# bnulwh/gpushare-scheduler-extender

Measured on AMD Instinct MI355X. Metric: pods bound/sec, higher is better.
Workload: dtype n/a

## Files before the change

native/engine/bindings.cc:

```cpp
#include <pybind11/pybind11.h>
#include <pybind11/stl.h>

#include <poll.h>
#include <pthread.h>
#include <sched.h>
#include <sys/eventfd.h>
#include <sys/timerfd.h>
#include <time.h>
#include <unistd.h>

#include <condition_variable>
#include <deque>
#include <memory>
#include <map>
#include <mutex>
#include <thread>

#include "allocstate.h"
#include "dpcore.h"
#include "h2.h"
#include "introspect.h"
#include "ledger.h"
#include "quantity.h"
#include "controller.h"
// ... 475 lines not shown
    d["unfiltered_binds"] = s.unfiltered_binds.load();
    d["live_gets"] = s.live_gets.load();
    d["qps_waits"] = s.qps_waits.load();
    d["moves_failed"] = s.moves_failed.load();
    d["physical_posts"] = s.physical_posts.load();
    d["plugin_auth_denied"] = s.plugin_auth_denied.load();
    d["token_reviews"] = s.token_reviews.load();
    d["backoffs"] = s.backoffs.load();
    d["publication_waits"] = s.publication_waits.load();
    d["physical_refused"] = s.physical_refused.load();
    d["epoch"] = srv_->epoch();
    d["api_throttled"] = srv_->api_throttled();
    d["api_throttle_wait_s"] = srv_->api_throttle_wait_s();
    auto hist = [](const LatencyHist& h) {
      py::dict o;
      py::list bounds, counts;
      for (int i = 0; i < LatencyHist::kBuckets; ++i) bounds.append(LatencyHist::kBounds[i]);
      for (int i = 0; i <= LatencyHist::kBuckets; ++i) counts.append(h.counts[i].load());
      o["bounds"] = bounds;
      o["counts"] = counts;
      o["n"] = h.n.load();
      o["sum"] = static_cast<double>(h.sum_ns.load()) / 1e9;
      return o;
    };
    d["filter_latency"] = hist(s.filter_lat);
    d["bind_latency"] = hist(s.bind_lat);
    d["api_latency"] = hist(s.api_lat);
    return d;
  }

  py::dict ledger_mutex() {
    introspect::MutexStats m = l_.mu().stats();
    py::dict d;
    d["acquisitions"] = m.acquisitions;
    d["contended"] = m.contended;
    d["wait_s"] = m.wait_s;
    d["max_wait_s"] = m.max_wait_s;
    d["hold_s"] = m.hold_s;
    d["max_hold_s"] = m.max_hold_s;
    return d;
  }

  void set_binds_enabled(bool on) {
    binds_enabled_ = on;
    if (srv_) srv_->set_binds_enabled(on);
  }

  py::list drain_annotation_repairs() {
    std::vector<AnnotationRepair> rs;
    {
      std::lock_guard<introspect::ProfiledMutex> g(l_.mu());
      rs = l_.drain_repairs();
    }
    py::list out;
    for (auto& a : rs) {
      py::dict d;
      d["uid"] = a.uid;
      d["namespace"] = a.ns;
      d["name"] = a.name;
      d["node"] = a.node;
      d["dev"] = a.dev;
      d["dev_total"] = a.dev_total;
      d["mem"] = a.mem;
      d["assume_ns"] = a.assume_ns;
      out.append(d);
    }
    return out;
  }

  void set_bind_order(const std::string& m) {
    if (m == "auto") {
      l_.set_order_mode(Ledger::kOrderAuto);
    } else if (m == "strict") {
      l_.set_order_mode(Ledger::kOrderStrict);
    } else if (m == "relaxed") {
      l_.set_order_mode(Ledger::kOrderRelaxed);
    } else {
      throw py::value_error("bind order must be auto, strict or relaxed");
    }
  }
  std::string bind_order() const { return Ledger::order_mode_name(l_.order_mode()); }

  void set_update_mode(bool on) {
    update_mode_ = on;
    if (srv_) srv_->set_update_mode(on);
  }

  py::list drain_bind_failures() {
    py::list out;
    if (!srv_) return out;
    for (auto& f : srv_->drain_failures()) {
      py::dict d;
      d["namespace"] = f.ns;
      d["name"] = f.name;
      d["uid"] = f.uid;
      d["node"] = f.node;
      d["message"] = f.message;
      out.append(d);
    }
    return out;
  }

  size_t pending_count() {
    std::lock_guard<introspect::ProfiledMutex> g(l_.mu());
    return l_.pending_count();
  }

  ~Engine() {
    stop_server();
    stop_controller();
  }

  PodView parse_pod(const py::bytes& b) {
    PodView v;
    std::string err;
    if (!parse_pod_bytes(b, l_.profile(), &v, &err)) throw py::value_error(err);
    return v;
  }

 private:
  Ledger l_;
  bool update_mode_ = false;
  std::unique_ptr<NativeServer> srv_;
  std::unique_ptr<Controller> ctl_;
  bool binds_enabled_ = true;
};

}

namespace {

class PyPodTracker {
 public:
  PyPodTracker(const py::dict& api, const std::string& ns, const std::string& label_selector)
      : t_(api_from(api), ns, label_selector) {}
  void start(double timeout) {
    std::string err;
    bool ok;
    {
      py::gil_scoped_release rel;
      ok = t_.start(timeout, &err);
    }
    if (!ok) throw std::runtime_error(err);
  }
  void stop() {
    py::gil_scoped_release rel;
    t_.stop();
  }
  std::string wait(const std::vector<std::string>& keys, int cond, double timeout) {
    py::gil_scoped_release rel;
    return t_.wait(keys, cond, timeout);
  }
  size_t size() const { return t_.size(); }

 private:
  PodTracker t_;
};

class PyReflectorProbe {
 public:
  PyReflectorProbe(const py::dict& api, const std::string& path, const std::string& field_selector, int page) {
    ReflectorConfig rc;
    rc.path = path;
    rc.field_selector = field_selector;
    rc.list_page_size = page;
    ReflectorHandler h;
    h.on_list = [this](const ListView& lv) {
      std::map<std::string, std::string> fresh;
      for (size_t k = 0; k < lv.size(); ++k) {
        std::string key, rv;
        if (key_rv(lv.doc(k), lv.obj(k), &key, &rv)) fresh[key] = rv;
      }
      std::lock_guard<std::mutex> g(mu_);
      view_.swap(fresh);
      lists_++;
    };
    h.on_event = [this](Ev ev, const json::Doc& d, uint32_t obj) {
      std::string key, rv;
      if (!key_rv(d, obj, &key, &rv)) return;
      std::lock_guard<std::mutex> g(mu_);
      if (ev == Ev::Deleted) {
        view_.erase(key);
      } else {
        view_[key] = rv;
      }
      events_++;
    };
    r_ = std::make_unique<Reflector>(api_from(api), rc, h);
  }
  ~PyReflectorProbe() { stop(); }
  void start() { r_->start(); }
  void stop() {
    if (r_) {
      py::gil_scoped_release rel;
      r_->stop();
    }
  }
  bool wait_synced(double t) {
    py::gil_scoped_release rel;
    return r_->wait_synced(t);
  }
  void request_relist() { r_->request_relist(); }
  py::dict view() {
    py::dict d;
    std::lock_guard<std::mutex> g(mu_);
    for (auto& kv : view_) d[py::str(kv.first)] = kv.second;
    return d;
  }
  py::dict stats() {
    py::dict d;
    d["relists"] = r_->relists();
    d["rewatches"] = r_->rewatches();
    d["errors"] = r_->errors();
    d["resource_version"] = r_->resource_version();
    std::lock_guard<std::mutex> g(mu_);
    d["lists"] = lists_;
    d["events"] = events_;
    return d;
  }

 private:
  static bool key_rv(const json::Doc& d, uint32_t obj, std::string* key, std::string* rv) {
    int64_t n = d.path(obj, {"metadata", "name"});
    if (n < 0) return false;
    int64_t ns = d.path(obj, {"metadata", "namespace"});
    int64_t r = d.path(obj, {"metadata", "resourceVersion"});
    *key = (ns >= 0 ? d.str(static_cast<uint32_t>(ns)) + "/" : std::string()) + d.str(static_cast<uint32_t>(n));
    *rv = r >= 0 ? d.str(static_cast<uint32_t>(r)) : std::string();
    return true;
  }
  std::unique_ptr<Reflector> r_;
  std::mutex mu_;
  std::map<std::string, std::string> view_;
  uint64_t lists_ = 0, events_ = 0;
};

class PyBatchClient {
 public:
  explicit PyBatchClient(const py::dict& api) : c_(api_from(api)) {}
  py::list run(const std::vector<std::tuple<std::string, std::string, py::bytes>>& reqs, int concurrency) {
    std::vector<std::tuple<std::string, std::string, std::string>> rq;
    rq.reserve(reqs.size());
    for (const auto& r : reqs) rq.emplace_back(std::get<0>(r), std::get<1>(r), std::string(std::get<2>(r)));
    std::vector<std::pair<int, std::string>> out;
    {
      py::gil_scoped_release rel;
      out = c_.run(rq, concurrency);
    }
    py::list l;
    for (auto& o : out) l.append(py::make_tuple(o.first, py::bytes(o.second)));
    return l;
  }

 private:
  BatchClient c_;
};

py::dict open_loop_run(const py::dict& api, const std::string& run, const std::string& pod_tmpl, double rate,
                       double duration_s, double warm_s, double hold_s, double drain_s, int creators, int deleters,
                       const std::string& ns, int grace) {
  OpenLoopConfig c;
  c.grace = grace;
  c.run = run;
  c.pod_tmpl = pod_tmpl;
  c.rate = rate;
  c.duration_s = duration_s;
  c.warm_s = warm_s;
  c.hold_s = hold_s;
  c.drain_s = drain_s;
  c.creators = creators;
  c.deleters = deleters;
  c.ns = ns;
  OpenLoop ol(api_from(api));
  std::vector<OpenLoopPod> pods;
  std::string err;
  int ce = 0, de = 0;
  bool ok;
  {
    py::gil_scoped_release rel;
    ok = ol.run(c, &pods, &err, &ce, &de);
  }
  if (!ok) throw std::runtime_error(err);
  py::list l;
  for (const auto& p : pods) l.append(py::make_tuple(p.arrival, p.created, p.bound, p.running, p.deleted, p.gone, p.failed));
  py::dict d;
  d["pods"] = l;
  d["create_errors"] = ce;
  d["delete_errors"] = de;
  return d;
}

class PyPodRuntime {
 public:
  PyPodRuntime(int dev, uint64_t arena_bytes, uint64_t arena_addr, uint64_t stream, uint64_t stride,
               const std::string& kernels_lib) {
    PodRuntimeConfig c;
    c.dev = dev;
    c.arena_bytes = arena_bytes;
    c.arena_addr = arena_addr;
    c.stream = reinterpret_cast<void*>(stream);
    c.stride = stride;
    c.kernels_lib = kernels_lib;
    r_ = std::make_unique<PodRuntime>(c);
    std::string err;
    if (!r_->init(&err)) throw std::runtime_error(err);
  }
// ... 727 lines not shown
  std::mutex fmu_;
  std::vector<Feed> feed_;
  std::vector<Waiting> waiting_;
  uint64_t waited_ = 0, feed_events_ = 0;
  double wait_s_ = 0, wait_max_s_ = 0;
  int tfd_ = -1;
  std::vector<std::thread> workers_;
  std::mutex wmu_;
  std::condition_variable wcv_;
  std::deque<std::unique_ptr<DpPending>> todo_, done_;
  std::deque<std::unique_ptr<DpPending>> todo_bg_;
  bool stopping_ = false;
  bool serving_on_ = false;
  int efd_ = -1;
  std::unique_ptr<DpCore> core_;
  std::unique_ptr<h2::Server> srv_;
  std::vector<std::tuple<uint64_t, std::string, std::string>> pending_;
  std::vector<DpEvent> events_;
  std::string device_list_, last_why_;
  bool have_list_ = false, fast_ = true;
  std::thread serving_;
  std::atomic<bool> stop_serving_{false};
  int pyfd_ = -1;
  double h_pref_s_ = 0, h_alloc_s_ = 0, h_pref_max_ = 0, h_alloc_max_ = 0;
  bool ready_ = true;
  bool preferred_ = false;
  double py_event_s_ = 0.002;
  double py_signal_at_ = 0, py_due_ = 0;
  bool py_deferred_ = false;
  double lock_wait_s_ = 0, lock_wait_max_s_ = 0;
  uint64_t lock_waits_ = 0;
  uint64_t h_pref_n_ = 0, h_alloc_n_ = 0;
  double spin_us_ = 1000;
  uint64_t calls_seen_ = 0;
  uint64_t spins_ = 0;
  uint64_t loop_iters_ = 0, spin_iters_ = 0;
  uint64_t passes_ = 0;
};

PYBIND11_MODULE(_engine, m) {
  m.def(
      "native_symbol", [](uint64_t pc) { return introspect::symbol_at(static_cast<uintptr_t>(pc)); },
      "Function name at a program counter of this process ('' when unknown).");
  m.def(
      "native_stacks",
      [](std::vector<int> tids, double timeout) {
        std::vector<introspect::Sample> got;
        {
          py::gil_scoped_release rel;
          got = introspect::capture(tids, timeout);
        }
        py::list out;
        for (auto& smp : got) out.append(py::make_tuple(smp.tid, smp.comm, smp.ok, smp.frames));
        return out;
      },
      py::arg("tids") = std::vector<int>(), py::arg("timeout") = 0.05,
      "Stack samples (tid, comm, ok, frames innermost-first) of this process's threads (all when tids is empty).");

  m.doc() = "gpushare MI355X native ledger engine";

  py::class_<PodView>(m, "PodView")
      .def(py::init<>())
      .def_readwrite("uid", &PodView::uid)
      .def_readwrite("name", &PodView::name)
      .def_readwrite("namespace", &PodView::ns)
      .def_readwrite("node", &PodView::node)
      .def_readwrite("phase", &PodView::phase)
      .def_readwrite("resource_version", &PodView::rv)
      .def_readwrite("deleting", &PodView::deleting)
      .def_readwrite("request", &PodView::request)
      .def_readwrite("dev_idx", &PodView::dev_idx)
      .def_readwrite("annot_mem", &PodView::annot_mem)
      .def_readwrite("has_annot_mem", &PodView::has_annot_mem)
      .def_readwrite("annot_dev_total", &PodView::annot_dev_total)
      .def_readwrite("assigned", &PodView::assigned)
      .def_readwrite("assume_time", &PodView::assume_time)
      .def_readwrite("cu_mask", &PodView::cu_mask)
      .def_readwrite("hold_idx", &PodView::hold_idx)
      .def_property_readonly("terminal", &PodView::terminal)
      .def_property_readonly("complete", &PodView::complete)
      .def_property_readonly("assigned_non_terminated", &PodView::assigned_non_terminated)
      .def("__repr__", [](const PodView& v) {
        return "<PodView " + v.ns + "/" + v.name + " uid=" + v.uid + " node=" + v.node +
               " req=" + std::to_string(v.request) + " idx=" + std::to_string(v.dev_idx) + ">";
      });

  py::class_<Engine>(m, "Engine")
      .def(py::init<const py::dict&>(), py::arg("profile") = py::dict())
      .def("profile", &Engine::profile)
      .def("upsert_node", &Engine::upsert_node, py::arg("name"), py::arg("total"), py::arg("count"),
           py::arg("dev_totals") = std::vector<int64_t>(), py::arg("address") = std::string())
      .def("upsert_node_json", &Engine::upsert_node_json)
      .def("remove_node", &Engine::remove_node)
      .def("has_node", &Engine::has_node)
      .def("node_info", &Engine::node_info)
      .def("upsert_pod", &Engine::upsert_pod)
      .def("remove_pod", &Engine::remove_pod)
      .def("known", &Engine::known)
      .def("pod_state", &Engine::pod_state)
      .def("upsert_pod_json", &Engine::upsert_pod_json)
      .def("check", &Engine::check)
      .def("filter", &Engine::filter)
      .def("prioritize", &Engine::prioritize)
      .def("assume", &Engine::assume)
      .def("finish_bind", &Engine::finish_bind, py::arg("uid"), py::arg("ok"), py::arg("ttl") = 30.0)
      .def("gc", &Engine::gc, py::arg("list_start") = 0.0)
      .def("assume_ordered", &Engine::assume_ordered, py::arg("uid"), py::arg("ns"), py::arg("name"),
           py::arg("node"), py::arg("req"), py::arg("cu_count") = std::string())
      .def("bind_blocked", &Engine::bind_blocked)
      .def("bind_wait", &Engine::bind_wait)
      .def("bind_leave", &Engine::bind_leave)
      .def("controller_gc", &Engine::controller_gc)
      .def("inspect", &Engine::inspect, py::arg("node") = std::string())
      .def("node_devices", &Engine::node_devices)
      .def("node_names", &Engine::node_names)
      .def("stats", &Engine::stats)
      .def("parse_pod", &Engine::parse_pod)
      .def("serve", &Engine::serve, py::arg("host"), py::arg("port"), py::arg("threads") = 2,
           py::arg("pool_threads") = 16, py::arg("fallback_port") = 0, py::arg("ttl") = 60.0,
           py::arg("api") = py::dict(), py::arg("update_mode") = false, py::arg("qps") = 0.0, py::arg("burst") = 10,
           py::arg("plugin_auth") = "none", py::arg("plugin_users") = std::vector<std::string>())
      .def("node_unaccounted", [](Engine& e, const std::string& node) { return e.node_unaccounted(node); })
      .def("begin_move", &Engine::begin_move, py::arg("uid"), py::arg("node"), py::arg("from_dev"), py::arg("to") = -1,
           py::arg("partner") = std::string(), py::arg("physical_on_to") = false, py::arg("req_hold") = -1,
           py::arg("req_hold_partner") = std::string())
      .def("end_move", &Engine::end_move)
      .def("set_unaccounted", &Engine::set_unaccounted, py::arg("node"), py::arg("extra"), py::arg("ttl") = 60.0)
      .def("begin_epoch", &Engine::begin_epoch)
      .def("publication_wait", &Engine::publication_wait)
      .def("stop_server", &Engine::stop_server)
      .def("start_controller", &Engine::start_controller, py::arg("api"), py::arg("resync") = 30.0,
           py::arg("sync_timeout") = 60.0, py::arg("watch_timeout") = 300)
      .def("stop_controller", &Engine::stop_controller)
      .def("controller_synced", &Engine::controller_synced)
      .def("controller_get_pod", &Engine::controller_get_pod)
      .def("controller_overcommitted", &Engine::controller_overcommitted)
      .def("controller_stats", &Engine::controller_stats)
      .def("server_stats", &Engine::server_stats)
      .def("ledger_mutex", &Engine::ledger_mutex)
      .def("drain_bind_failures", &Engine::drain_bind_failures)
      .def("set_binds_enabled", &Engine::set_binds_enabled)
      .def("set_update_mode", &Engine::set_update_mode)
      .def("set_bind_order", &Engine::set_bind_order)
      .def_property_readonly("bind_order", &Engine::bind_order)
      .def("drain_annotation_repairs", &Engine::drain_annotation_repairs)
      .def("pending_count", &Engine::pending_count);

  py::class_<PyPodTracker>(m, "PodTracker")
      .def(py::init<const py::dict&, const std::string&, const std::string&>(), py::arg("api"),
           py::arg("namespace") = std::string(), py::arg("label_selector") = std::string())
      .def("start", &PyPodTracker::start, py::arg("timeout") = 30.0)
      .def("stop", &PyPodTracker::stop)
      .def("wait", &PyPodTracker::wait, py::arg("keys"), py::arg("cond"), py::arg("timeout") = 120.0)
      .def("size", &PyPodTracker::size);
  m.attr("TRACK_BOUND") = static_cast<int>(PodTracker::Bound);
  m.attr("TRACK_RUNNING") = static_cast<int>(PodTracker::Running);
  m.attr("TRACK_GONE") = static_cast<int>(PodTracker::Gone);
  m.attr("TRACK_STOPPED") = static_cast<int>(PodTracker::Stopped);
  py::class_<PyReflectorProbe>(m, "ReflectorProbe")
      .def(py::init<const py::dict&, const std::string&, const std::string&, int>(), py::arg("api"),
           py::arg("path") = "/api/v1/pods", py::arg("field_selector") = "", py::arg("page") = 500)
      .def("start", &PyReflectorProbe::start)
      .def("stop", &PyReflectorProbe::stop)
      .def("wait_synced", &PyReflectorProbe::wait_synced, py::arg("timeout") = 10.0)
      .def("request_relist", &PyReflectorProbe::request_relist)
      .def("view", &PyReflectorProbe::view)
      .def("stats", &PyReflectorProbe::stats);

  m.def("open_loop_run", &open_loop_run, py::arg("api"), py::arg("run"), py::arg("pod_tmpl"), py::arg("rate"),
        py::arg("duration_s") = 2.0, py::arg("warm_s") = 0.5, py::arg("hold_s") = 0.0, py::arg("drain_s") = 20.0,
        py::arg("creators") = 16, py::arg("deleters") = 16, py::arg("ns") = "default", py::arg("grace") = -1);
  py::class_<PyBatchClient>(m, "BatchClient")
      .def(py::init<const py::dict&>())
      .def("run", &PyBatchClient::run, py::arg("requests"), py::arg("concurrency") = 8);

  py::class_<PyPodRuntime>(m, "PodRuntime")
      .def(py::init<int, uint64_t, uint64_t, uint64_t, uint64_t, const std::string&>(), py::arg("dev"),
           py::arg("arena_bytes"), py::arg("arena_addr") = 0, py::arg("stream") = 0, py::arg("stride") = 1 << 20,
           py::arg("kernels_lib") = std::string())
      .def("serve", &PyPodRuntime::serve, py::arg("host") = "127.0.0.1", py::arg("port") = 0,
           py::arg("cpus") = std::vector<int>())
      .def("stop", &PyPodRuntime::stop)
      .def("admit", &PyPodRuntime::admit, py::arg("uid"), py::arg("bytes"), py::arg("verify") = true)
      .def("release", &PyPodRuntime::release)
      .def("verify", &PyPodRuntime::verify)
      .def("stats", &PyPodRuntime::stats);


  py::class_<CuPartitioner>(m, "CuPartitioner")
      .def(py::init<int, int>(), py::arg("cu_count") = 256, py::arg("xcc_count") = 8)
      .def("allocate", [](CuPartitioner& c, const std::string& uid, int n) {
             std::vector<int> out;
             std::string err;
             if (!c.allocate(uid, n, &out, &err)) throw py::value_error(err);
             return out;
           }, py::call_guard<AllocLock>())
      .def("release", &CuPartitioner::release, py::call_guard<AllocLock>())
      .def("adopt", &CuPartitioner::adopt, py::call_guard<AllocLock>())
      .def("swap_owners", &CuPartitioner::swap_owners, py::call_guard<AllocLock>())
      .def("holds", &CuPartitioner::holds, py::call_guard<AllocLock>())
      .def("held_by", &CuPartitioner::held_by, py::call_guard<AllocLock>())
      .def("held", [](const CuPartitioner& c) {
        py::dict d;
        for (const auto& kv : c.held()) d[py::str(kv.first)] = kv.second;
        return d;
      }, py::call_guard<AllocLock>())
      .def("free_count", &CuPartitioner::free_count, py::call_guard<AllocLock>())
      .def_property_readonly("cu_count", &CuPartitioner::cu_count)
      .def_property_readonly("xcc_count", &CuPartitioner::xcc_count);
  m.def("cu_words", &cu_words, py::call_guard<AllocLock>());
  m.def("parse_cu_words", [](const std::string& w) {
    try {
      return parse_cu_words(w);
    } catch (const std::invalid_argument& e) {
      throw py::value_error(e.what());
    }
  }, py::call_guard<AllocLock>());
  m.def("cu_ranges", &cu_ranges, py::call_guard<AllocLock>());

  py::class_<AllocPod>(m, "AllocPod")
      .def(py::init<>())
      .def_readwrite("uid", &AllocPod::uid)
      .def_readwrite("key", &AllocPod::key)
      .def_readwrite("namespace", &AllocPod::ns)
      .def_readwrite("name", &AllocPod::name)
      .def_readwrite("rv", &AllocPod::rv)
      .def_readwrite("phase", &AllocPod::phase)
      .def_readwrite("creation", &AllocPod::creation)
      .def_readwrite("node", &AllocPod::node)
      .def_readwrite("dev", &AllocPod::dev)
      .def_readwrite("request", &AllocPod::request)
      .def_readwrite("containers", &AllocPod::containers)
      .def_readwrite("assume_time", &AllocPod::assume_time)
      .def_readwrite("dev_total", &AllocPod::dev_total)
      .def_readwrite("assigned", &AllocPod::assigned)
      .def_readwrite("complete", &AllocPod::complete)
      .def_readwrite("terminating", &AllocPod::terminating)
      .def_readwrite("term_grace_s", &AllocPod::term_grace_s)
      .def_readwrite("cu_count", &AllocPod::cu_count)
      .def_readwrite("cu_mask", &AllocPod::cu_mask)
      .def_readwrite("hold_idx", &AllocPod::hold_idx)
      .def_readwrite("hold_partner", &AllocPod::hold_partner)
      .def_readwrite("raw", &AllocPod::raw)
      .def_property_readonly("pending", &AllocPod::pending);

  auto rec_dict = [](const AllocRecord& r) {
    py::dict d;
    d["aid"] = r.aid;
    d["ids"] = r.ids;
    d["uid"] = r.uid;
    d["dev"] = r.dev;
    d["units"] = r.units;
    d["cu_mask"] = r.cu_mask;
    d["owner"] = r.owner;
    d["t"] = r.t;
    d["iso"] = r.iso;
    d["on_gpu"] = r.on_gpu;
    return d;
  };
  py::class_<AllocState>(m, "AllocState")
      .def(py::init([](const std::string& node, const std::vector<std::tuple<int, int, int>>& devs) {
             std::vector<std::pair<int, std::pair<int, int>>> d;
             for (const auto& t : devs) d.push_back({std::get<0>(t), {std::get<1>(t), std::get<2>(t)}});
             return new AllocState(node, d);
           }),
           py::arg("node"), py::arg("devices"))
      .def("observe", &AllocState::observe, py::call_guard<AllocLock>())
      .def("release", &AllocState::release, py::call_guard<AllocLock>())
      .def("deleted", &AllocState::deleted, py::arg("uid"), py::arg("now") = -1.0, py::call_guard<AllocLock>())
      .def("lingering", &AllocState::lingering, py::call_guard<AllocLock>())
      .def("gone_held", &AllocState::gone_held, py::call_guard<AllocLock>())
      .def("set_linger", &AllocState::set_linger, py::call_guard<AllocLock>())
      .def("set_skip_partners", &AllocState::set_skip_partners, py::call_guard<AllocLock>())
      .def("linger_enabled", &AllocState::linger_enabled, py::call_guard<AllocLock>())
      .def("linger_count", &AllocState::linger_count, py::call_guard<AllocLock>())
      .def("is_tombstoned", &AllocState::is_tombstoned, py::call_guard<AllocLock>())
      .def("resync", [](AllocState& s, const std::vector<std::string>& live, double now) {
        s.resync(std::unordered_set<std::string>(live.begin(), live.end()), now);
      }, py::arg("live"), py::arg("now") = -1.0, py::call_guard<AllocLock>())
      .def("holders", &AllocState::holders, py::call_guard<AllocLock>())
      .def("has_pod", [](const AllocState& s, const std::string& uid) { return s.pod(uid) != nullptr; }, py::call_guard<AllocLock>())
      .def("uid_for_key", [](const AllocState& s, const std::string& key) -> std::string {
        const AllocPod* p = s.pod_by_key(key);
        return p ? p->uid : std::string();
      }, py::call_guard<AllocLock>())
      .def("pod_view", [](const AllocState& s, const std::string& uid) -> py::object {
             const AllocPod* p = s.pod(uid);
             if (!p) return py::none();
             py::dict d;
             d["rv"] = p->rv;
             d["phase"] = p->phase;
             d["dev"] = p->dev;
             d["assigned"] = p->assigned;
             d["cu_mask"] = p->cu_mask;
             d["hold_idx"] = p->hold_idx;
             d["hold_partner"] = p->hold_partner;
             return d;
           }, py::call_guard<AllocLock>())
      .def("pod_views", [](const AllocState& s) {
        std::vector<AllocPod> copy;
        {
          AllocLock lock;
          copy.resize(s.pods().size());
          size_t i = 0;
          for (const auto& kv : s.pods()) {
            const AllocPod& p = kv.second;
            AllocPod& c = copy[i++];
// ... 244 lines not shown
```

native/engine/podruntime.cc:

```cpp
#include "podruntime.h"

#include <dlfcn.h>

#include <algorithm>
#include <cstdio>
#include <set>
#include <vector>

#include "json.h"

namespace gsx {

namespace {

constexpr uint64_t kAlign = 2ull << 20;

uint64_t tag_of(const std::string& uid) {
  uint64_t h = 1469598103934665603ull;
  for (unsigned char c : uid) {
    h ^= c;
    h *= 1099511628211ull;
  }
  return h | 1;
}

struct GsxSlice {
  uint64_t addr, bytes, tag;
};

}

PodRuntime::PodRuntime(PodRuntimeConfig cfg) : cfg_(std::move(cfg)) {}

PodRuntime::~PodRuntime() {
  stop();
  if (lib_) dlclose(lib_);
}

bool PodRuntime::init(std::string* err) {
  if (!cfg_.arena_addr) return true;
  lib_ = dlopen(cfg_.kernels_lib.c_str(), RTLD_NOW | RTLD_LOCAL);
  if (!lib_) {
    *err = std::string("dlopen ") + cfg_.kernels_lib + ": " + dlerror();
    return false;
  }
  set_device_ = reinterpret_cast<int (*)(int)>(dlsym(lib_, "gsx_set_device"));
  admit_n_ = reinterpret_cast<int (*)(void*, const void*, int, int, int, uint64_t, uint64_t*)>(
      dlsym(lib_, "gsx_hbm_admit_n"));
  last_error_ = reinterpret_cast<const char* (*)()>(dlsym(lib_, "gsx_last_error"));
  if (!set_device_ || !admit_n_ || !last_error_) {
    *err = "libgsx_kernels.so lacks gsx_set_device / gsx_hbm_admit_n";
    return false;
  }
  if (!cfg_.stream || cfg_.stride < 16 || cfg_.stride % 16) {
    *err = "pod runtime needs a stream and a 16-B multiple stamp stride";
    return false;
  }
  return true;
}

int PodRuntime::serve(const std::string& host, int port, std::string* err, std::vector<int> cpus) {
  srv_ = std::make_unique<CtlServer>([this](const http::Message& m) { return handle(m); });
  srv_->set_cpus(std::move(cpus));
  return srv_->start(host, port, err);
}

void PodRuntime::stop() {
  if (srv_) srv_->stop();
}

uint64_t PodRuntime::resident_bytes() const {
  std::lock_guard<std::mutex> g(mu_);
  uint64_t b = 0;
  for (auto& kv : slices_) b += kv.second.size;
  return b;
}

size_t PodRuntime::resident() const {
  std::lock_guard<std::mutex> g(mu_);
  return slices_.size();
}

int64_t PodRuntime::run_admit(bool stamp, const std::string& uid, bool verify, std::string* err) {
  if (!cfg_.arena_addr) return 0;
  std::vector<GsxSlice> sl;
  auto add = [&](const Slice& s) {
    for (auto& e : s.ext) sl.push_back(GsxSlice{cfg_.arena_addr + e.first, e.second, s.tag});
  };
  auto mine = slices_.find(uid);
  if (mine != slices_.end()) add(mine->second);
  const int n_stamp = stamp ? static_cast<int>(sl.size()) : 0;
  if (verify) {
    for (auto& kv : slices_) {
      if (kv.first != uid) add(kv.second);
    }
  }
  if (sl.empty()) return 0;
  uint64_t bad = 0;
  int rc = set_device_(cfg_.dev);
  if (rc == 0) rc = admit_n_(cfg_.stream, sl.data(), static_cast<int>(sl.size()), n_stamp, 1, cfg_.stride, &bad);
  if (rc != 0) {
    *err = std::string("gsx_hbm_admit_n: ") + last_error_();
    return -1;
  }
  return static_cast<int64_t>(bad);
}

bool PodRuntime::carve_locked(const std::string& uid, uint64_t bytes, std::string* err) {
  uint64_t size = (bytes + kAlign - 1) / kAlign * kAlign;
  std::vector<std::pair<uint64_t, uint64_t>> used;
  for (auto& kv : slices_) used.insert(used.end(), kv.second.ext.begin(), kv.second.ext.end());
  std::sort(used.begin(), used.end());
  Slice s{{}, size, tag_of(uid)};
  uint64_t pos = 0, need = size;
  auto take = [&](uint64_t end) {
    if (need && end > pos) {
      uint64_t n = std::min(need, end - pos);
      s.ext.emplace_back(pos, n);
      need -= n;
    }
  };
  for (auto& u : used) {
    take(u.first);
    pos = std::max(pos, u.first + u.second);
  }
  take(cfg_.arena_bytes);
  if (need) {
    *err = "arena exhausted: need " + std::to_string(size) + " B, " + std::to_string(size - need) + " free of " +
           std::to_string(cfg_.arena_bytes);
    return false;
  }
  slices_[uid] = std::move(s);
  return true;
}

void PodRuntime::admit_group_locked(const std::vector<Pending*>& group) {
  std::vector<Pending*> fresh, again;
  bool verify_all = false;
  for (Pending* p : group) {
    if (slices_.count(p->uid)) {
      again.push_back(p);
    } else if (!carve_locked(p->uid, p->bytes, &p->err)) {
      failed_++;
      p->result = -1;
      continue;
    } else {
      fresh.push_back(p);
    }
    verify_all = verify_all || p->verify;
  }
  if (fresh.empty() && again.empty()) return;
  std::vector<GsxSlice> sl;
  std::set<std::string> listed;
  for (Pending* p : fresh) {
    for (auto& e : slices_[p->uid].ext) sl.push_back(GsxSlice{cfg_.arena_addr + e.first, e.second, slices_[p->uid].tag});
    listed.insert(p->uid);
  }
  const int n_stamp = static_cast<int>(sl.size());
  for (auto& kv : slices_) {
    if (listed.count(kv.first)) continue;
    bool own = false;
    for (Pending* p : again) own = own || p->uid == kv.first;
    if (!verify_all && !own) continue;
    for (auto& e : kv.second.ext) sl.push_back(GsxSlice{cfg_.arena_addr + e.first, e.second, kv.second.tag});
  }
  uint64_t bad = 0;
  int rc = 0;
  if (cfg_.arena_addr && !sl.empty()) {
    rc = set_device_(cfg_.dev);
    if (rc == 0) rc = admit_n_(cfg_.stream, sl.data(), static_cast<int>(sl.size()), n_stamp, 1, cfg_.stride, &bad);
    batches_++;
  }
  if (rc != 0) {
    std::string e = std::string("gsx_hbm_admit_n: ") + last_error_();
    for (Pending* p : fresh) {
      slices_.erase(p->uid);
      failed_++;
      p->result = -1;
      p->err = e;
    }
    for (Pending* p : again) {
      p->result = -1;
      p->err = e;
    }
    return;
  }
  bad_ += bad;
  auto own_bad = [&](Pending* p) -> int64_t {
    if (p->verify || bad == 0) return static_cast<int64_t>(bad);
    std::vector<GsxSlice> mine;
    auto it = slices_.find(p->uid);
    if (it == slices_.end()) return 0;
    for (auto& e : it->second.ext) mine.push_back(GsxSlice{cfg_.arena_addr + e.first, e.second, it->second.tag});
    uint64_t b = 0;
    if (!mine.empty() && admit_n_(cfg_.stream, mine.data(), static_cast<int>(mine.size()), 0, 1, cfg_.stride, &b) != 0) {
      return static_cast<int64_t>(bad);
    }
    return static_cast<int64_t>(b);
  };
  for (Pending* p : fresh) {
    admitted_++;
    p->result = own_bad(p);
  }
  for (Pending* p : again) p->result = own_bad(p);
}

int64_t PodRuntime::admit(const std::string& uid, uint64_t bytes, bool verify, std::string* err) {
  Pending me{uid, bytes, verify};
  std::unique_lock<std::mutex> q(qmu_);
  queue_.push_back(&me);
  while (!me.done) {
    if (leading_) {
      qcv_.wait(q);
      continue;
    }
    leading_ = true;
    std::vector<Pending*> group;
    group.swap(queue_);
    q.unlock();
    try {
      std::lock_guard<std::mutex> g(mu_);
      admit_group_locked(group);
    } catch (const std::exception& e) {
      for (Pending* p : group) {
        if (p->result >= 0 && p->err.empty()) {
          p->result = -1;
          p->err = std::string("admission: ") + e.what();
        }
      }
    }
    q.lock();
    for (Pending* p : group) p->done = true;
    leading_ = false;
    qcv_.notify_all();
  }
  if (me.result < 0) *err = me.err;
  return me.result;
}

bool PodRuntime::release(const std::string& uid) {
  std::lock_guard<std::mutex> g(mu_);
  return slices_.erase(uid) > 0;
}

int64_t PodRuntime::verify_all(std::string* err) {
  std::lock_guard<std::mutex> g(mu_);
  return run_admit(false, std::string(), true, err);
}

CtlServer::Reply PodRuntime::handle(const http::Message& m) {
  CtlServer::Reply rep;
  std::string_view path = m.path();
  const std::string_view pre = "/v1/pods/";
  if (path.substr(0, pre.size()) == pre && path.size() > pre.size()) {
    std::string uid(path.substr(pre.size()));
    if (m.method == "POST") {
      json::Doc d;
      std::string err;
      int64_t bytes = 0;
      bool verify = true;
      if (d.parse(m.body, &err)) {
        int64_t b = d.find(0, "bytes");
        if (b >= 0) d.as_int(static_cast<uint32_t>(b), &bytes);
        int64_t v = d.find(0, "verify");
        if (v >= 0) verify = d.at(static_cast<uint32_t>(v)).type != json::T::False;
      }
      if (bytes <= 0) {
        rep.status = 400;
        rep.body = "{\"error\":\"bytes must be > 0\"}";
        return rep;
      }
      int64_t bad = admit(uid, static_cast<uint64_t>(bytes), verify, &err);
      if (bad < 0) {
        rep.status = 409;
        rep.body = "{\"error\":";
        json::append_quoted(&rep.body, err);
        rep.body.push_back('}');
        return rep;
      }
      rep.body = "{\"bad\":" + std::to_string(bad) + "}";
      return rep;
    }
    if (m.method == "DELETE") {
      rep.status = release(uid) ? 200 : 404;
      return rep;
    }
  }
  if (m.method == "GET" && path == "/v1/stats") {
    std::lock_guard<std::mutex> g(mu_);
    char b[256];
    std::snprintf(b, sizeof(b),
                  "{\"admitted\":%llu,\"failed\":%llu,\"bad\":%llu,\"resident\":%zu,\"batches\":%llu,\"native\":true}",
                  (unsigned long long)admitted_, (unsigned long long)failed_, (unsigned long long)bad_,
                  slices_.size(), (unsigned long long)batches_);
    rep.body = b;
    return rep;
  }
  rep.status = 404;
  rep.body = "{\"error\":\"not found\"}";
  return rep;
}

}
```

native/engine/podruntime.h:

```cpp
#pragma once

#include <cstdint>
#include <condition_variable>
#include <map>
#include <memory>
#include <mutex>
#include <string>
#include <utility>
#include <vector>

#include "ctlserver.h"

namespace gsx {

struct PodRuntimeConfig {
  int dev = 0;
  uint64_t arena_bytes = 0;
  uint64_t arena_addr = 0;
  void* stream = nullptr;
  uint64_t stride = 1 << 20;
  std::string kernels_lib;
};

class PodRuntime {
 public:
  explicit PodRuntime(PodRuntimeConfig cfg);
  ~PodRuntime();
  bool init(std::string* err);
  int serve(const std::string& host, int port, std::string* err, std::vector<int> cpus = {});
  void stop();
  int64_t admit(const std::string& uid, uint64_t bytes, bool verify, std::string* err);
  bool release(const std::string& uid);
  int64_t verify_all(std::string* err);
  uint64_t admitted() const { return admitted_; }
  uint64_t failed() const { return failed_; }
  uint64_t bad() const { return bad_; }
  uint64_t batches() const { return batches_; }
  uint64_t resident_bytes() const;
  size_t resident() const;

 private:
  struct Slice {
    std::vector<std::pair<uint64_t, uint64_t>> ext;
    uint64_t size, tag;
  };
  CtlServer::Reply handle(const http::Message& m);
  int64_t run_admit(bool stamp, const std::string& uid, bool verify, std::string* err);
  struct Pending {
    std::string uid;
    uint64_t bytes;
    bool verify;
    bool done = false;
    int64_t result = 0;
    std::string err;
  };
  bool carve_locked(const std::string& uid, uint64_t bytes, std::string* err);
  void admit_group_locked(const std::vector<Pending*>& group);

  PodRuntimeConfig cfg_;
  mutable std::mutex mu_;
  std::map<std::string, Slice> slices_;
  uint64_t admitted_ = 0, failed_ = 0, bad_ = 0, batches_ = 0;
  std::mutex qmu_;
  std::condition_variable qcv_;
  std::vector<Pending*> queue_;
  bool leading_ = false;
  std::unique_ptr<CtlServer> srv_;
  void* lib_ = nullptr;
  int (*set_device_)(int) = nullptr;
  int (*admit_n_)(void*, const void*, int, int, int, uint64_t, uint64_t*) = nullptr;
  const char* (*last_error_)() = nullptr;
};

}
```

native/engine/tracker.cc:

```cpp
#include "tracker.h"

#include <algorithm>
#include <atomic>
#include <chrono>
#include <deque>
#include <thread>
#include <unordered_set>

namespace gsx {

namespace {

std::string str_at(const json::Doc& d, int64_t i) { return i >= 0 ? d.str(static_cast<uint32_t>(i)) : std::string(); }

}

PodTracker::PodTracker(const ApiConfig& cfg, const std::string& ns, const std::string& label_selector) {
  ReflectorConfig rc;
  rc.path = ns.empty() ? "/api/v1/pods" : "/api/v1/namespaces/" + ns + "/pods";
  rc.label_selector = label_selector;
  ReflectorHandler h;
  auto key_of = [](const json::Doc& d, uint32_t obj) {
    std::string ns_ = str_at(d, d.path(obj, {"metadata", "namespace"}));
    std::string name = str_at(d, d.path(obj, {"metadata", "name"}));
    return ns_.empty() ? name : ns_ + "/" + name;
  };
  h.on_list = [this, key_of](const ListView& lv) {
    std::lock_guard<std::mutex> g(mu_);
    pods_.clear();
    for (size_t k = 0; k < lv.size(); ++k) {
      const json::Doc& d = lv.doc(k);
      uint32_t i = lv.obj(k);
      St& s = pods_[key_of(d, i)];
      s.node = str_at(d, d.path(i, {"spec", "nodeName"}));
      s.phase = str_at(d, d.path(i, {"status", "phase"}));
    }
    cv_.notify_all();
  };
  h.on_event = [this, key_of](Ev ev, const json::Doc& d, uint32_t obj) {
    std::string key = key_of(d, obj);
    std::lock_guard<std::mutex> g(mu_);
    if (ev == Ev::Deleted) {
      pods_.erase(key);
    } else {
      St& s = pods_[key];
      s.node = str_at(d, d.path(obj, {"spec", "nodeName"}));
      s.phase = str_at(d, d.path(obj, {"status", "phase"}));
    }
    cv_.notify_all();
  };
  r_ = std::make_unique<Reflector>(cfg, rc, h);
}

PodTracker::~PodTracker() { stop(); }

bool PodTracker::start(double timeout_s, std::string* err) {
  r_->start();
  if (!r_->wait_synced(timeout_s)) {
    *err = "tracker did not sync: " + r_->last_error();
    return false;
  }
  return true;
}

void PodTracker::stop() {
  if (r_) r_->stop();
  cv_.notify_all();
}

size_t PodTracker::size() const {
  std::lock_guard<std::mutex> g(mu_);
  return pods_.size();
}

bool PodTracker::ok_locked(const std::string& key, int cond, std::string* err) const {
  auto it = pods_.find(key);
  switch (cond) {
    case Bound:
      return it != pods_.end() && !it->second.node.empty();
    case Running:
      if (it != pods_.end() && it->second.phase == "Failed") *err = "pod " + key + " Failed";
      return it != pods_.end() && it->second.phase == "Running";
    case Stopped:
      return it == pods_.end() || it->second.phase == "Succeeded" || it->second.phase == "Failed";
    default:
      return it == pods_.end();
  }
}

std::string PodTracker::wait(const std::vector<std::string>& keys, int cond, double timeout_s) {
  auto deadline = std::chrono::steady_clock::now() + std::chrono::duration<double>(timeout_s);
  std::unique_lock<std::mutex> lk(mu_);
  size_t i = 0;
  while (true) {
    std::string err;
    while (i < keys.size() && ok_locked(keys[i], cond, &err)) ++i;
    if (!err.empty()) return err;
    if (i == keys.size()) return std::string();
    if (cv_.wait_until(lk, deadline) == std::cv_status::timeout) {
      while (i < keys.size() && ok_locked(keys[i], cond, &err)) ++i;
      if (i == keys.size()) return std::string();
      return "timeout: " + std::to_string(keys.size() - i) + " pods not " +
             (cond == Bound ? "bound" : cond == Running ? "Running" : cond == Stopped ? "stopped" : "gone") + ", e.g. " + keys[i];
    }
  }
}

BatchClient::~BatchClient() {
  {
    std::lock_guard<std::mutex> g(mu_);
    stop_ = true;
  }
  cv_.notify_all();
  for (auto& t : helpers_) t.join();
}

void BatchClient::work_on(const std::vector<Req>& reqs, std::vector<std::pair<int, std::string>>* out) {
  while (true) {
    size_t i = next_.fetch_add(1);
    if (i >= reqs.size()) return;
    int status = 0;
    std::string body, err;
    const auto& r = reqs[i];
    if (api_.request(std::get<0>(r), std::get<1>(r), std::get<2>(r), "application/json", &status, &body, &err)) {
      (*out)[i] = {status, std::move(body)};
    } else {
      (*out)[i] = {-1, err};
    }
  }
}

void BatchClient::helper(int me) {
  uint64_t seen = 0;
  std::unique_lock<std::mutex> lk(mu_);
  while (true) {
    cv_.wait(lk, [&] { return stop_ || (gen_ != seen && me < want_); });
    if (stop_) return;
    seen = gen_;
    const std::vector<Req>* reqs = reqs_;
    auto* out = out_;
    ++busy_;
    lk.unlock();
    work_on(*reqs, out);
    lk.lock();
    if (--busy_ == 0) done_cv_.notify_all();
  }
}

std::vector<std::pair<int, std::string>> BatchClient::run(const std::vector<Req>& reqs, int concurrency) {
  std::lock_guard<std::mutex> one(run_mu_);
  std::vector<std::pair<int, std::string>> out(reqs.size());
  const int n = std::max(1, std::min<int>(concurrency, static_cast<int>(reqs.size())));
  {
    std::lock_guard<std::mutex> g(mu_);
    while (static_cast<int>(helpers_.size()) < n - 1) {
      const int k = static_cast<int>(helpers_.size());
      helpers_.emplace_back([this, k] { helper(k); });
    }
    reqs_ = &reqs;
    out_ = &out;
    next_.store(0);
    want_ = n - 1;
    ++gen_;
  }
  if (n > 1) cv_.notify_all();
  work_on(reqs, &out);
  std::unique_lock<std::mutex> lk(mu_);
  done_cv_.wait(lk, [&] { return busy_ == 0; });
  want_ = 0;
  reqs_ = nullptr;
  out_ = nullptr;
  return out;
}

}

namespace gsx {

namespace {
double mono() { return std::chrono::duration<double>(std::chrono::steady_clock::now().time_since_epoch()).count(); }
}

bool OpenLoop::run(const OpenLoopConfig& c, std::vector<OpenLoopPod>* pods, std::string* err, int* create_errors,
                   int* delete_errors) {
  const size_t n = static_cast<size_t>(std::max(1.0, c.rate * c.duration_s));
  pods->assign(n, OpenLoopPod{});
  std::mutex mu;
  std::condition_variable cv;
  std::deque<std::pair<double, size_t>> dq;
  std::atomic<int> cerr{0}, derr{0};
  std::atomic<size_t> next{0}, gone{0};
  std::atomic<bool> stop{false};
  const std::string prefix = "ol-" + c.run + "-";
  auto index_of = [&](const json::Doc& d, uint32_t obj) -> int64_t {
    std::string name = str_at(d, d.path(obj, {"metadata", "name"}));
    if (name.compare(0, prefix.size(), prefix) != 0) return -1;
    char* e = nullptr;
    long long i = std::strtoll(name.c_str() + prefix.size(), &e, 10);
    return (e && *e == '\0' && i >= 0 && static_cast<size_t>(i) < n) ? i : -1;
  };
  auto observe = [&](Ev ev, const json::Doc& d, uint32_t obj) {
    int64_t i = index_of(d, obj);
    if (i < 0) return;
    const double now = mono();
    std::lock_guard<std::mutex> g(mu);
    OpenLoopPod& p = (*pods)[static_cast<size_t>(i)];
    if (ev == Ev::Deleted) {
      if (p.gone == 0) {
        p.gone = now;
        gone.fetch_add(1);
        cv.notify_all();
      }
      return;
    }
    if (p.bound == 0 && !str_at(d, d.path(obj, {"spec", "nodeName"})).empty()) p.bound = now;
    std::string phase = str_at(d, d.path(obj, {"status", "phase"}));
    if (p.running == 0 && (phase == "Running" || phase == "Failed")) {
      p.running = now;
      p.failed = phase == "Failed";
      dq.emplace_back(now + c.hold_s, static_cast<size_t>(i));
      cv.notify_all();
    }
  };
  ReflectorConfig rc;
  rc.path = "/api/v1/namespaces/" + c.ns + "/pods";
  rc.label_selector = c.label_key + "=" + c.run;
  ReflectorHandler h;
  h.on_list = [&](const ListView& lv) {
    for (size_t k = 0; k < lv.size(); ++k) observe(Ev::Modified, lv.doc(k), lv.obj(k));
  };
  h.on_event = [&](Ev ev, const json::Doc& d, uint32_t obj) { observe(ev, d, obj); };
  Reflector r(cfg_, rc, h);
  r.start();
  if (!r.wait_synced(30)) {
    *err = "open-loop watch did not sync: " + r.last_error();
    r.stop();
    return false;
  }
  const std::string coll = "/api/v1/namespaces/" + c.ns + "/pods";
  const double t0 = mono() + 0.01;
  std::vector<std::thread> th;
  for (int k = 0; k < std::max(1, c.creators); ++k) {
    th.emplace_back([&] {
      ApiClient api(cfg_);
      std::string body, resp, e;
      while (!stop.load()) {
        size_t i = next.fetch_add(1);
        if (i >= n) return;
        const double at = t0 + static_cast<double>(i) / c.rate;
        const double wait = at - mono();
        if (wait > 0) std::this_thread::sleep_for(std::chrono::duration<double>(wait));
        body = c.pod_tmpl;
// ... 62 lines not shown
```

native/engine/tracker.h:

```cpp
#pragma once

#include <atomic>
#include <condition_variable>
#include <memory>
#include <mutex>
#include <string>
#include <thread>
#include <tuple>
#include <unordered_map>
#include <vector>

#include "apiclient.h"
#include "informer.h"

namespace gsx {

class PodTracker {
 public:
  enum Cond : int { Bound = 0, Running = 1, Gone = 2, Stopped = 3 };
  PodTracker(const ApiConfig& cfg, const std::string& ns, const std::string& label_selector);
  ~PodTracker();
  bool start(double timeout_s, std::string* err);
  void stop();
  std::string wait(const std::vector<std::string>& keys, int cond, double timeout_s);
  size_t size() const;

 private:
  struct St {
    std::string node, phase;
  };
  bool ok_locked(const std::string& key, int cond, std::string* err) const;

  std::unique_ptr<Reflector> r_;
  mutable std::mutex mu_;
  std::condition_variable cv_;
  std::unordered_map<std::string, St> pods_;
};

struct OpenLoopConfig {
  std::string ns = "default";
  std::string label_key = "gsx-ol";
  std::string run;
  std::string pod_tmpl;
  double rate = 1000;
  double duration_s = 2.0;
  double warm_s = 0.5;
  double hold_s = 0.0;
  double drain_s = 20.0;
  int creators = 16, deleters = 16;
  int grace = -1;
};

struct OpenLoopPod {
  double arrival = 0, created = 0, bound = 0, running = 0, deleted = 0, gone = 0;
  bool failed = false;
};

class OpenLoop {
 public:
  explicit OpenLoop(const ApiConfig& cfg) : cfg_(cfg) {}
  bool run(const OpenLoopConfig& c, std::vector<OpenLoopPod>* pods, std::string* err, int* create_errors,
           int* delete_errors);

 private:
  ApiConfig cfg_;
};

class BatchClient {
 public:
  using Req = std::tuple<std::string, std::string, std::string>;
  explicit BatchClient(const ApiConfig& cfg) : api_(cfg) {}
  ~BatchClient();
  std::vector<std::pair<int, std::string>> run(const std::vector<Req>& reqs, int concurrency);

 private:
  void work_on(const std::vector<Req>& reqs, std::vector<std::pair<int, std::string>>* out);
  void helper(int me);

  ApiClient api_;
  std::mutex run_mu_, mu_;
  std::condition_variable cv_, done_cv_;
  std::vector<std::thread> helpers_;
  const std::vector<Req>* reqs_ = nullptr;
  std::vector<std::pair<int, std::string>>* out_ = nullptr;
  std::atomic<size_t> next_{0};
  uint64_t gen_ = 0;
  int want_ = 0, busy_ = 0;
  bool stop_ = false;
};

}
```

native/kernels/hbm_stamp.hip:

```cpp
#include <hip/hip_runtime.h>

#include <algorithm>
#include <mutex>

#include "gsx_internal.h"
#include "gsx_kernels.h"

using namespace gsx;

namespace {

struct alignas(16) Stamp {
  uint64_t tag;
  uint64_t off;
};
typedef unsigned long long u64x2 __attribute__((ext_vector_type(2)));

typedef const __attribute__((address_space(1))) u64x2* global_stamp_ptr;

typedef __attribute__((address_space(1))) u64x2* global_stamp_wptr;

__device__ __forceinline__ u64x2 load_stamp(const char* p) { return *(global_stamp_ptr)(p); }
__device__ __forceinline__ void store_stamp(char* p, uint64_t tag, uint64_t off) {
  u64x2 v;
  v.x = tag;
  v.y = off;
  *(global_stamp_wptr)(p) = v;
}

__device__ __forceinline__ void stamp_extent(const gsx_slice sl, uint64_t stride) {
  const uint64_t n = sl.bytes / stride;
  char* base = reinterpret_cast<char*>(sl.addr);
  for (uint64_t i = blockIdx.x * 256ull + threadIdx.x; i < n; i += gridDim.x * 256ull) {
    store_stamp(base + i * stride, sl.tag, i * stride);
  }
}

__device__ __forceinline__ void count_bad_stamps(const gsx_slice sl, uint64_t stride, unsigned long long* bad) {
  const uint64_t n = sl.bytes / stride;
  const char* base = reinterpret_cast<const char*>(sl.addr);
  uint32_t mine = 0;
  for (uint64_t i = blockIdx.x * 256ull + threadIdx.x; i < n; i += gridDim.x * 256ull) {
    const u64x2 st = load_stamp(base + i * stride);
    mine += (st.x != sl.tag || st.y != i * stride) ? 1u : 0u;
  }
  for (int o = 32; o > 0; o >>= 1) mine += __shfl_xor(mine, o, 64);
  if ((threadIdx.x & 63) == 0 && mine) atomicAdd_system(bad, static_cast<unsigned long long>(mine));
}

constexpr int kMaxSlices = 32;
struct SliceTable {
  gsx_slice s[kMaxSlices];
  int n;
};

__global__ __launch_bounds__(256) void stamp_slices_kernel(SliceTable t, uint64_t stride) {
  stamp_extent(t.s[blockIdx.y], stride);
}

__global__ __launch_bounds__(256) void verify_slices_kernel(SliceTable t, uint64_t stride, unsigned long long* bad) {
  count_bad_stamps(t.s[blockIdx.y], stride, bad);
}


std::mutex g_mu;
unsigned long long* g_host_counter[kMaxDevices] = {nullptr};
std::mutex g_dev_mu[kMaxDevices];

int pinned_counter(const char* who, int* dev, unsigned long long** hc) {
  if (int rc = current_device(who, dev)) return rc;
  std::lock_guard<std::mutex> g(g_mu);
  if (!g_host_counter[*dev]) {
    GSX_CHECK(hipHostMalloc(reinterpret_cast<void**>(&g_host_counter[*dev]), 64, hipHostMallocCoherent));
  }
  *hc = g_host_counter[*dev];
  return 0;
}

constexpr int kTableBlocks = 1024, kRangeBlocks = 8192;

int launch(const char* who, hipStream_t st, const gsx_slice* slices, int n_stamp, int n_verify, uint64_t stride,
           int max_blocks, bool sync, uint64_t* bad) {
  auto tables = [&](int count, auto&& kernel) {
    for (int from = 0; from < count; from += kMaxSlices) {
      SliceTable t;
      t.n = std::min(kMaxSlices, count - from);
      uint64_t maxn = 0;
      for (int i = 0; i < t.n; ++i) {
        t.s[i] = slices[from + i];
        maxn = std::max<uint64_t>(maxn, t.s[i].bytes / stride);
      }
      const uint64_t gx = std::clamp<uint64_t>((maxn + 255) / 256, 1, max_blocks);
      kernel(dim3(static_cast<uint32_t>(gx), t.n), t);
      GSX_CHECK(hipGetLastError());
    }
    return 0;
  };
  if (int rc = tables(n_stamp, [&](dim3 grid, const SliceTable& t) {
        hipLaunchKernelGGL(stamp_slices_kernel, grid, dim3(256), 0, st, t, stride);
      }))
    return rc;
  if (!n_verify) {
    if (sync) GSX_CHECK(hipStreamSynchronize(st));
    return 0;
  }
  int dev = 0;
  unsigned long long* hc = nullptr;
  if (int rc = pinned_counter(who, &dev, &hc)) return rc;
  std::lock_guard<std::mutex> dl(g_dev_mu[dev]);
  __atomic_store_n(hc, 0ull, __ATOMIC_SEQ_CST);
  if (int rc = tables(n_verify, [&](dim3 grid, const SliceTable& t) {
        hipLaunchKernelGGL(verify_slices_kernel, grid, dim3(256), 0, st, t, stride, hc);
      }))
    return rc;
  GSX_CHECK(hipStreamSynchronize(st));
  *bad = __atomic_load_n(hc, __ATOMIC_SEQ_CST);
  return 0;
}

}

extern "C" {

int gsx_hbm_stamp(void* stream, void* base, uint64_t bytes, uint64_t stride, uint64_t tag) {
  if (!base || stride < sizeof(Stamp) || stride % 16) return fail_arg("gsx_hbm_stamp: stride must be >=16, %16");
  if (reinterpret_cast<uintptr_t>(base) % 16) return fail_arg("gsx_hbm_stamp: base not 16-B aligned");
  if (bytes < stride) return 0;
  const gsx_slice sl = {reinterpret_cast<uintptr_t>(base), bytes, tag};
  return launch("gsx_hbm_stamp", S(stream), &sl, 1, 0, stride, kRangeBlocks, false, nullptr);
}

int gsx_hbm_verify(void* stream, const void* base, uint64_t bytes, uint64_t stride, uint64_t tag, uint64_t* bad) {
  if (!base || stride < sizeof(Stamp) || stride % 16) return fail_arg("gsx_hbm_verify: stride must be >=16, %16");
  if (reinterpret_cast<uintptr_t>(base) % 16) return fail_arg("gsx_hbm_verify: base not 16-B aligned");
  *bad = 0;
  if (bytes < stride) return 0;
  const gsx_slice sl = {reinterpret_cast<uintptr_t>(base), bytes, tag};
  return launch("gsx_hbm_verify", S(stream), &sl, 0, 1, stride, kRangeBlocks, true, bad);
}

int gsx_hbm_admit_n(void* stream, const gsx_slice* slices, int n, int n_stamp, int verify, uint64_t stride,
                    uint64_t* bad) {
  *bad = 0;
  if (n < 0 || n_stamp < 0 || n_stamp > n || stride < sizeof(Stamp) || stride % 16)
    return fail_arg("gsx_hbm_admit_n: bad n/n_stamp/stride");
  for (int i = 0; i < n; ++i) {
    if (!slices[i].addr || slices[i].addr % 16) return fail_arg("gsx_hbm_admit_n: slice base not 16-B aligned");
  }
  return launch("gsx_hbm_admit_n", S(stream), slices, n_stamp, verify ? n : 0, stride, kTableBlocks, true, bad);
}

}
```

Baseline: 11680.

## Release runtime lock during GPU admit and wake tracker waiters selectively

PodRuntime now drops its state mutex while the HBM admit kernel runs and caches the selected device per endpoint thread, so it no longer calls set_device on every batch. PodTracker records which keys waiters are blocked on and notifies the condition variable only when an event satisfies or errors one of them, replacing a notify_all on every event. The pinned-counter lookup becomes a lock-free atomic fast path. Event and wakeup counters are also exposed through the Python bindings. Releasing mu_ mid-admit lets other threads change slices_ concurrently, which adds a risk of races.

```diff
diff --git a/native/engine/bindings.cc b/native/engine/bindings.cc
--- a/native/engine/bindings.cc
+++ b/native/engine/bindings.cc
@@ -651,6 +651,13 @@
     return t_.wait(keys, cond, timeout);
   }
   size_t size() const { return t_.size(); }
+  py::dict stats() const {
+    PodTracker::Stats s = t_.stats();
+    py::dict d;
+    d["events"] = s.events;
+    d["wakeups"] = s.wakeups;
+    return d;
+  }
 
  private:
   PodTracker t_;
@@ -1684,7 +1691,8 @@
       .def("start", &PyPodTracker::start, py::arg("timeout") = 30.0)
       .def("stop", &PyPodTracker::stop)
       .def("wait", &PyPodTracker::wait, py::arg("keys"), py::arg("cond"), py::arg("timeout") = 120.0)
-      .def("size", &PyPodTracker::size);
+      .def("size", &PyPodTracker::size)
+      .def("stats", &PyPodTracker::stats);
   m.attr("TRACK_BOUND") = static_cast<int>(PodTracker::Bound);
   m.attr("TRACK_RUNNING") = static_cast<int>(PodTracker::Running);
   m.attr("TRACK_GONE") = static_cast<int>(PodTracker::Gone);
diff --git a/native/engine/podruntime.cc b/native/engine/podruntime.cc
--- a/native/engine/podruntime.cc
+++ b/native/engine/podruntime.cc
@@ -27,6 +27,9 @@
 struct GsxSlice {
   uint64_t addr, bytes, tag;
 };
+
+thread_local bool t_endpoint = false;
+thread_local int t_dev = -1;
 
 }
 
@@ -134,7 +137,7 @@
   return true;
 }
 
-void PodRuntime::admit_group_locked(const std::vector<Pending*>& group) {
+void PodRuntime::admit_group(const std::vector<Pending*>& group, std::unique_lock<std::mutex>& lk) {
   std::vector<Pending*> fresh, again;
   bool verify_all = false;
   for (Pending* p : group) {
@@ -166,13 +169,19 @@
   }
   uint64_t bad = 0;
   int rc = 0;
+  std::string e;
   if (cfg_.arena_addr && !sl.empty()) {
-    rc = set_device_(cfg_.dev);
+    lk.unlock();
+    if (!t_endpoint || t_dev != cfg_.dev) {
+      rc = set_device_(cfg_.dev);
+      t_dev = rc == 0 ? cfg_.dev : -1;
+    }
     if (rc == 0) rc = admit_n_(cfg_.stream, sl.data(), static_cast<int>(sl.size()), n_stamp, 1, cfg_.stride, &bad);
+    if (rc != 0) e = std::string("gsx_hbm_admit_n: ") + last_error_();
+    lk.lock();
     batches_++;
   }
   if (rc != 0) {
-    std::string e = std::string("gsx_hbm_admit_n: ") + last_error_();
     for (Pending* p : fresh) {
       slices_.erase(p->uid);
       failed_++;
@@ -219,8 +228,8 @@
     group.swap(queue_);
     q.unlock();
     try {
-      std::lock_guard<std::mutex> g(mu_);
-      admit_group_locked(group);
+      std::unique_lock<std::mutex> g(mu_);
+      admit_group(group, g);
     } catch (const std::exception& e) {
       for (Pending* p : group) {
         if (p->result >= 0 && p->err.empty()) {
@@ -250,6 +259,7 @@
 
 CtlServer::Reply PodRuntime::handle(const http::Message& m) {
   CtlServer::Reply rep;
+  t_endpoint = true;
   std::string_view path = m.path();
   const std::string_view pre = "/v1/pods/";
   if (path.substr(0, pre.size()) == pre && path.size() > pre.size()) {
diff --git a/native/engine/podruntime.h b/native/engine/podruntime.h
--- a/native/engine/podruntime.h
+++ b/native/engine/podruntime.h
@@ -55,7 +55,7 @@
     std::string err;
   };
   bool carve_locked(const std::string& uid, uint64_t bytes, std::string* err);
-  void admit_group_locked(const std::vector<Pending*>& group);
+  void admit_group(const std::vector<Pending*>& group, std::unique_lock<std::mutex>& lk);
 
   PodRuntimeConfig cfg_;
   mutable std::mutex mu_;
diff --git a/native/engine/tracker.cc b/native/engine/tracker.cc
--- a/native/engine/tracker.cc
+++ b/native/engine/tracker.cc
@@ -47,7 +47,14 @@
       s.node = str_at(d, d.path(obj, {"spec", "nodeName"}));
       s.phase = str_at(d, d.path(obj, {"status", "phase"}));
     }
-    cv_.notify_all();
+    ++events_;
+    for (const Awaited& a : awaited_) {
+      std::string err;
+      if (*a.key == key && (ok_locked(key, a.cond, &err) || !err.empty())) {
+        cv_.notify_all();
+        break;
+      }
+    }
   };
   r_ = std::make_unique<Reflector>(cfg, rc, h);
 }
@@ -71,6 +78,11 @@
 size_t PodTracker::size() const {
   std::lock_guard<std::mutex> g(mu_);
   return pods_.size();
+}
+
+PodTracker::Stats PodTracker::stats() const {
+  std::lock_guard<std::mutex> g(mu_);
+  return Stats{events_, wakeups_};
 }
 
 bool PodTracker::ok_locked(const std::string& key, int cond, std::string* err) const {
@@ -97,7 +109,17 @@
     while (i < keys.size() && ok_locked(keys[i], cond, &err)) ++i;
     if (!err.empty()) return err;
     if (i == keys.size()) return std::string();
-    if (cv_.wait_until(lk, deadline) == std::cv_status::timeout) {
+    awaited_.push_back(Awaited{&keys[i], cond});
+    const std::cv_status st = cv_.wait_until(lk, deadline);
+    for (size_t k = 0; k < awaited_.size(); ++k) {
+      if (awaited_[k].key == &keys[i] && awaited_[k].cond == cond) {
+        awaited_[k] = awaited_.back();
+        awaited_.pop_back();
+        break;
+      }
+    }
+    if (st == std::cv_status::no_timeout) ++wakeups_;
+    if (st == std::cv_status::timeout) {
       while (i < keys.size() && ok_locked(keys[i], cond, &err)) ++i;
       if (i == keys.size()) return std::string();
       return "timeout: " + std::to_string(keys.size() - i) + " pods not " +
diff --git a/native/engine/tracker.h b/native/engine/tracker.h
--- a/native/engine/tracker.h
+++ b/native/engine/tracker.h
@@ -24,10 +24,19 @@
   void stop();
   std::string wait(const std::vector<std::string>& keys, int cond, double timeout_s);
   size_t size() const;
+  struct Stats {
+    uint64_t events;
+    uint64_t wakeups;
+  };
+  Stats stats() const;
 
  private:
   struct St {
     std::string node, phase;
+  };
+  struct Awaited {
+    const std::string* key;
+    int cond;
   };
   bool ok_locked(const std::string& key, int cond, std::string* err) const;
 
@@ -35,6 +44,8 @@
   mutable std::mutex mu_;
   std::condition_variable cv_;
   std::unordered_map<std::string, St> pods_;
+  std::vector<Awaited> awaited_;
+  uint64_t events_ = 0, wakeups_ = 0;
 };
 
 struct OpenLoopConfig {
diff --git a/native/kernels/hbm_stamp.hip b/native/kernels/hbm_stamp.hip
--- a/native/kernels/hbm_stamp.hip
+++ b/native/kernels/hbm_stamp.hip
@@ -1,6 +1,7 @@
 #include <hip/hip_runtime.h>
 
 #include <algorithm>
+#include <atomic>
 #include <mutex>
 
 #include "gsx_internal.h"
@@ -64,16 +65,19 @@
 
 
 std::mutex g_mu;
-unsigned long long* g_host_counter[kMaxDevices] = {nullptr};
+std::atomic<unsigned long long*> g_host_counter[kMaxDevices];
 std::mutex g_dev_mu[kMaxDevices];
 
 int pinned_counter(const char* who, int* dev, unsigned long long** hc) {
   if (int rc = current_device(who, dev)) return rc;
+  *hc = g_host_counter[*dev].load(std::memory_order_acquire);
+  if (*hc) return 0;
   std::lock_guard<std::mutex> g(g_mu);
-  if (!g_host_counter[*dev]) {
-    GSX_CHECK(hipHostMalloc(reinterpret_cast<void**>(&g_host_counter[*dev]), 64, hipHostMallocCoherent));
+  *hc = g_host_counter[*dev].load(std::memory_order_relaxed);
+  if (!*hc) {
+    GSX_CHECK(hipHostMalloc(reinterpret_cast<void**>(hc), 64, hipHostMallocCoherent));
+    g_host_counter[*dev].store(*hc, std::memory_order_release);
   }
-  *hc = g_host_counter[*dev];
   return 0;
 }
 
```

Result: slower. 8982 (-23.1%).
